# davrempe/contact-human-dynamics

Hardware: NVIDIA H100
Metric: optimised frames/sec (batched phys-optim) (higher is better)
Workload: dtype f64

## Files before the change

### contact-human-dynamics_b200/csrc/chd_api.cu

```cuda
#include <cuda_runtime.h>

#include <cstdio>
#include <cstdlib>
#include <cstring>
#include <vector>

#include "../../include/chd.h"
#include "chd_dev.h"

__global__ void chd_k_stage_begin(ChdDev D);
__global__ void chd_k_eval(ChdDev D);
__global__ void chd_k_init(ChdDev D);
__global__ void chd_k_kkt(ChdDev D);
__global__ void chd_k_kkt_gwin(ChdDev D);
__global__ void chd_k_kcopy(ChdDev D);
__global__ void chd_k_curv(ChdDev D);
__global__ void chd_k_asm(ChdDev D);
__global__ void chd_k_fp64_peak(int mode, int iters, double* sink);
__global__ void chd_k_hess_base(ChdDev D);
__global__ void chd_k_hess_dur(ChdDev D);
__global__ void chd_k_hess_zero(ChdDev D);
__global__ void chd_k_hess_fin(ChdDev D, int mode);
__global__ void chd_k_tables(ChdDev D);
__global__ void chd_k_clear_dyn(ChdDev D);
// ... 155 lines not shown
      chd_k_hess_dur<<<dim3(8, B), CHD_THREADS, 0, b->copy_stream>>>(b->D);
      chd_k_hess_fin<<<B, 128, 0, b->copy_stream>>>(b->D, 1);
      b->launches += 2;
    }
    chd_k_curv<<<dim3(8, B), 256, 0, b->copy_stream>>>(b->D);
    b->launches++;
    CHD_CUDA(cudaEventRecord(b->ev_copy, b->copy_stream));
    {
      Timer t(b, KT_SAMPLE);
      chd_k_snapshot<<<B, 128, 0, b->stream>>>(b->D, b->d_frames);
    }
    if ((it % check_every) == check_every - 1) {
      CHD_CUDA(cudaMemcpyAsync(b->h_ipm, b->D.ipm, B * sizeof(ChdIpm), cudaMemcpyDeviceToHost, b->stream));
      CHD_CUDA(cudaStreamSynchronize(b->stream));
      bool any = false;
      for (int i = 0; i < B; ++i) any |= (b->h_ipm[i].phase != CHD_PH_FINISHED);
      if (!any) break;
    }
  }
  CHD_CUDA(cudaMemcpyAsync(b->h_ipm, b->D.ipm, B * sizeof(ChdIpm), cudaMemcpyDeviceToHost, b->stream));
  CHD_CUDA(cudaStreamSynchronize(b->stream));
  CHD_CUDA(cudaStreamSynchronize(b->copy_stream));
  CHD_CUDA(cudaGetLastError());
  return 0;
}

}

extern "C" {

const char* chd_version(void) { return "libchd 0.1 (sm_90a)"; }

int chd_measure_fp64_peak(double* dfma_gflops, double* dmma_gflops) {
  int dev = 0, sms = 0;
  CHD_CUDA(cudaGetDevice(&dev));
  CHD_CUDA(cudaDeviceGetAttribute(&sms, cudaDevAttrMultiProcessorCount, dev));
  double* sink = nullptr;
  CHD_CUDA(cudaMalloc((void**)&sink, sizeof(double) * 1024));
  cudaEvent_t e0, e1;
  CHD_CUDA(cudaEventCreate(&e0));
  CHD_CUDA(cudaEventCreate(&e1));
  const int blocks = sms * 8, threads = 256, iters = 4096;
  for (int mode = 0; mode < 2; ++mode) {
    float best = 1e30f;
    for (int rep = 0; rep < 4; ++rep) {
      CHD_CUDA(cudaEventRecord(e0));
      chd_k_fp64_peak<<<blocks, threads>>>(mode, iters, sink);
      CHD_CUDA(cudaEventRecord(e1));
      CHD_CUDA(cudaEventSynchronize(e1));
      float ms = 0;
      CHD_CUDA(cudaEventElapsedTime(&ms, e0, e1));
      if (rep > 0 && ms < best) best = ms;
    }
    const double flop = mode == 0 ? (double)blocks * threads * iters * 8 * 2 : (double)blocks * (threads / 32) * iters * 4 * 512;
    double* out = mode == 0 ? dfma_gflops : dmma_gflops;
    if (out) *out = flop / (best * 1e-3) / 1e9;
  }
  cudaEventDestroy(e0), cudaEventDestroy(e1), cudaFree(sink);
  return 0;
}

static int batch_create_impl(const chd_phys_problem* problems, int32_t batch, const chd_phys_weights* weights, int32_t device,
                             const chd_phys_options& opt, chd_phys_batch* b);

int chd_phys_batch_create(const chd_phys_problem* problems, int32_t batch, const chd_phys_weights* weights, int32_t device,
                          const chd_phys_options* opt, chd_phys_batch** out) {
  if (!problems || batch <= 0 || !out) return -1;
  chd_phys_options o = {-1};
  if (opt) o = *opt;
  if (o.stage3_band_above < -1 || o.stage3_band_above > CHD_MAX_DUR) return -1;
  chd_phys_batch* b = new chd_phys_batch();
  std::memset(&b->D, 0, sizeof(b->D));
  const int rc = batch_create_impl(problems, batch, weights, device, o, b);
  if (rc) {
    chd_phys_batch_destroy(b);
    return rc;
  }
  *out = b;
  return 0;
}

static int batch_create_impl(const chd_phys_problem* problems, int32_t batch, const chd_phys_weights* weights, int32_t device,
                             const chd_phys_options& opt, chd_phys_batch* b) {
  const bool host_only = device == -2;
  if (device >= 0) CHD_CUDA(cudaSetDevice(device));
  chd_phys_weights w = {0.4, 1.7, 0.3, 0.1, 0.1};
  if (weights) w = *weights;
  int rc = chd_build_layout(problems, batch, w, b->hb, opt.stage3_band_above);
  if (rc) return rc;
  ChdHostBatch& hb = b->hb;
  ChdDev& D = b->D;
  std::memset(&D, 0, sizeof(D));
  b->host_only = host_only;
  if (host_only) return 0;
  D.B = hb.B, D.S = hb.S, D.Pmax = hb.Pmax, D.n_max = hb.n_max, D.m_max = hb.m_max, D.slots_max = hb.slots_max;
  D.sets_max = hb.sets_max, D.tab_max = hb.tab_max, D.F_max = hb.F_max, D.Kd_max = hb.Kd_max, D.Kr_max = hb.Kr_max;
  D.Na_max = hb.Na_max, D.nb_max = hb.nb_max, D.w_max = hb.w_max, D.par_stride = hb.par_stride(), D.n_ee_max = hb.n_ee_max;
  D.fo_max = hb.fo_max, D.Ph_max = hb.Ph_max;
  CHD_CUDA(cudaStreamCreate(&b->stream));
  {
    int dev_id = 0;
    cudaMemPool_t pool;
    CHD_CUDA(cudaGetDevice(&dev_id));
    CHD_CUDA(cudaDeviceGetDefaultMemPool(&pool, dev_id));
    unsigned long long keep = ~0ull;
    CHD_CUDA(cudaMemPoolSetAttribute(pool, cudaMemPoolAttrReleaseThreshold, &keep));
  }
// ... 174 lines not shown

int chd_phys_get_ent_col(const chd_phys_batch* b, int32_t* ent_col) {
  if (!b || !ent_col) return -1;
  if (b->host_only) {
    std::memcpy(ent_col, b->hb.ent_col.data(), b->hb.ent_col.size() * sizeof(int));
    return 0;
  }
  CHD_CUDA(cudaStreamSynchronize(b->stream));
  CHD_CUDA(cudaMemcpy(ent_col, b->D.ent_col, b->hb.ent_col.size() * sizeof(int), cudaMemcpyDeviceToHost));
  return 0;
}

int chd_phys_get_duals(const chd_phys_batch* b, double* y, double* zL, double* zU, double* s, double* row_scale, double* obj_scale) {
  if (!b || b->host_only) return -1;
  const size_t B = b->hb.B, mm = B * b->hb.m_max;
  CHD_CUDA(cudaStreamSynchronize(b->stream));
  if (y) CHD_CUDA(cudaMemcpy(y, b->D.y, mm * sizeof(double), cudaMemcpyDeviceToHost));
  if (zL) CHD_CUDA(cudaMemcpy(zL, b->D.zL, mm * sizeof(double), cudaMemcpyDeviceToHost));
  if (zU) CHD_CUDA(cudaMemcpy(zU, b->D.zU, mm * sizeof(double), cudaMemcpyDeviceToHost));
  if (s) CHD_CUDA(cudaMemcpy(s, b->D.s, mm * sizeof(double), cudaMemcpyDeviceToHost));
  if (row_scale) CHD_CUDA(cudaMemcpy(row_scale, b->D.sc, mm * sizeof(double), cudaMemcpyDeviceToHost));
  if (obj_scale) {
    std::vector<ChdIpm> ipm(B);
    CHD_CUDA(cudaMemcpy(ipm.data(), b->D.ipm, B * sizeof(ChdIpm), cudaMemcpyDeviceToHost));
    for (size_t i = 0; i < B; ++i) obj_scale[i] = ipm[i].sf;
  }
  return 0;
}

int chd_phys_stage_stats(const chd_phys_batch* b, double* stats) {
  if (!b || !stats || b->host_only || !b->h_ipm) return -1;
  const int B = b->hb.B;
  for (int s = 0; s < 6; ++s)
    for (int i = 0; i < B; ++i)
      for (int q = 0; q < 4; ++q) stats[((size_t)s * B + i) * 4 + q] = b->h_ipm[i].st_stat[s][q];
  return 0;
}

int chd_phys_solve_stage(chd_phys_batch* b, int32_t stage, int32_t max_iter, int32_t* status, int32_t* iters, double* stats) {
  if (!b || stage < 0 || stage > 5 || b->host_only) return -1;
  const int B = b->hb.B;
  int sched[1] = {stage};
  int rc = set_schedule(b, sched, 1, stage, max_iter);
  if (rc) return rc;
  if ((rc = run_schedule(b))) return rc;
  for (int i = 0; i < B; ++i) {
    const ChdIpm& I = b->h_ipm[i];
    if (status) status[i] = I.st_status[stage];
    if (iters) iters[i] = I.st_iters[stage];
    if (stats) {
      double* s = stats + 8 * i;
      s[0] = I.f, s[1] = I.E0, s[2] = I.viol_u, s[3] = I.dual_u, s[4] = I.compl_u, s[5] = I.mu, s[6] = I.delta_w, s[7] = I.ls_fail;
    }
    if (i == 0 && getenv("CHD_PROF")) fprintf(stderr, "chd prof (Mcycles) seq0 stage %d: err %.2f asm %.2f factor %.2f border %.2f back %.2f rec %.2f\n", stage, I.prof[0]/1e6, I.prof[1]/1e6, I.prof[2]/1e6, I.prof[3]/1e6, I.prof[4]/1e6, I.prof[5]/1e6);
  }
  return 0;
}

int chd_phys_sample_device(chd_phys_batch* b, double* out_device, void* stream) {
  if (!b || !out_device || b->host_only) return -1;
  cudaStream_t st = stream ? (cudaStream_t)stream : b->stream;
  if (st == b->stream) {
    Timer t(b, KT_SAMPLE);
    chd_k_sample<<<b->hb.B, 128, 0, st>>>(b->D, out_device, b->d_frames);
    return 0;
  }
  cudaEvent_t ev;
  CHD_CUDA(cudaEventCreateWithFlags(&ev, cudaEventDisableTiming));
  CHD_CUDA(cudaEventRecord(ev, b->stream));
  CHD_CUDA(cudaStreamWaitEvent(st, ev, 0));
  chd_k_sample<<<b->hb.B, 128, 0, st>>>(b->D, out_device, b->d_frames);
  CHD_CUDA(cudaEventRecord(ev, st));
  CHD_CUDA(cudaStreamWaitEvent(b->stream, ev, 0));
  CHD_CUDA(cudaEventDestroy(ev));
  return 0;
}

int chd_phys_sample(chd_phys_batch* b, double* out, int32_t* frames_out) {
  if (!b || !out || b->host_only) return -1;
  const ChdHostBatch& hb = b->hb;
  const size_t stride = 6 + 7 * (size_t)hb.n_ee_max, cnt = (size_t)hb.B * hb.fo_max * stride;
  CHD_CUDA(cudaMemsetAsync(b->d_samples, 0, cnt * sizeof(double), b->stream));
  int rc = chd_phys_sample_device(b, b->d_samples, nullptr);
  if (rc) return rc;
  CHD_CUDA(cudaMemcpyAsync(out, b->d_samples, cnt * sizeof(double), cudaMemcpyDeviceToHost, b->stream));
  if (frames_out) CHD_CUDA(cudaMemcpyAsync(frames_out, b->d_frames, hb.B * sizeof(int), cudaMemcpyDeviceToHost, b->stream));
  CHD_CUDA(cudaStreamSynchronize(b->stream));
  return 0;
}

int chd_phys_solve(chd_phys_batch* b, double* samples, int32_t* frames_out, int32_t* success, int32_t* stage_status,
                   int32_t* stage_iters) {
  if (!b || b->host_only) return -1;
  const ChdHostBatch& hb = b->hb;
  const int B = hb.B;
  const size_t stride = 6 + 7 * (size_t)hb.n_ee_max, snap = (size_t)B * hb.fo_max * stride;
  int sched[6] = {CHD_STAGE_11, CHD_STAGE_12, CHD_STAGE_21, CHD_STAGE_22, CHD_STAGE_3, CHD_STAGE_4};
  int rc = set_schedule(b, sched, 6, -1, 0);
  if (rc) return rc;
  if (samples) CHD_CUDA(cudaMemsetAsync(b->D.snapshots, 0, 3 * snap * sizeof(double), b->stream));
  if ((rc = run_schedule(b))) return rc;
  for (int i = 0; i < B; ++i) {
    const ChdIpm& I = b->h_ipm[i];
    if (success) success[2 * i] = I.st_status[CHD_STAGE_22] == 0, success[2 * i + 1] = I.st_status[CHD_STAGE_3] == 0 || I.st_status[CHD_STAGE_4] == 0;
    for (int s = 0; s < 6; ++s) {
      if (stage_status) stage_status[(size_t)s * B + i] = I.st_status[s];
      if (stage_iters) stage_iters[(size_t)s * B + i] = I.st_iters[s];
// ... 39 lines not shown
```

### contact-human-dynamics_b200/csrc/chd_kkt.cu

```cuda
#include <cuda_runtime.h>

#include "chd_block.cuh"
#include "chd_eval.cuh"
#include "chd_kkt_tiles.cuh"

__device__ __forceinline__ void chd_hess_sample(const ChdCtx& c, const ChdKT& K, const int* vk, int s, const ChdSpl* P, const double* sign, int np,
                                                int deriv, double wgt, int lane, double* ws) {
  const bool tau = c.opt_dur && s >= 2 && deriv == 0;
  if (lane < 28) {
    const int pa = lane / 14, q = lane % 14;
    double v0 = 0.0, v1 = 0.0, v2 = 0.0;
    int ia = -1;
    if (pa < np) {
      if (q < 12) {
        const int va = P[pa].var[q];
        const double wa = sign[pa] * chd_slot_w(P[pa], deriv, q);
        if (va >= 0 && wa != 0.0) {
          ia = vk[va];
          v0 = q % 3 == 0 ? wa : 0.0, v1 = q % 3 == 1 ? wa : 0.0, v2 = q % 3 == 2 ? wa : 0.0;
        }
      } else if (tau) {
        ChdTau u;
        chd_spl_tau(c, s, s - 2, P[pa], u);
        const int var = q == 12 ? u.va : u.vb;
// ... 434 lines not shown
  if (E0 <= CHD_TOL && violu <= CHD_CONSTR_VIOL_TOL && dual_u <= CHD_DUAL_INF_TOL && compl_u <= CHD_COMPL_INF_TOL) new_status = 0, done = true;
  else if (I.iter >= I.max_iter) new_status = -1, done = true;
  if (!done) {
    const double mu_min = fmin(CHD_TOL, CHD_COMPL_INF_TOL) / (CHD_KAPPA_EPS + 1.0);
    while (true) {
      const double Emu = fmax(fmax(dual_inf / s_d, cviol), compl_err(mu) / s_c);
      if (Emu <= CHD_KAPPA_EPS * mu && mu > mu_min) mu = fmax(mu_min, fmin(CHD_KAPPA_MU * mu, pow(mu, CHD_THETA_MU)));
      else break;
    }
  }
  __syncthreads();
  if (tid == 0) {
    I.f = D.cost[2 * b];
    I.E0 = E0, I.viol_u = violu, I.dual_u = dual_u, I.compl_u = compl_u;
    I.status = new_status;
    s_fail = 0;
    if (done) chd_stage_advance(D, I, new_status, c.sg.snap_after);
    if (!done) {
      I.mu = mu;
      I.tau = fmax(CHD_TAU_MIN, 1.0 - mu);
      if (I.iter == 0) I.theta_max = 1e4 * fmax(1.0, theta), I.theta_min = 1e-4 * fmax(1.0, theta), I.theta_ref = theta;
      if (mu != I.mu_filter) I.nfilt = 0, I.mu_filter = mu;
      I.theta0 = theta;
    }
  }
  if (done) return true;
  c.mu = mu;
  c.tau = fmax(CHD_TAU_MIN, 1.0 - mu);
  c.polish = E0 <= CHD_TOL && dual_u <= CHD_DUAL_INF_TOL && compl_u <= CHD_COMPL_INF_TOL && violu > CHD_CONSTR_VIOL_TOL &&
             I.delta_w < CHD_DW_POLISH;
  c.delta_w = c.polish ? CHD_DW_POLISH : I.delta_w;
  return false;
}

__device__ __forceinline__ void chd_kkt_assemble(const ChdDev& D, const ChdKktCtx& c) {
  const ChdIpm& I = *c.I;
  const ChdKT& K = c.K;
  const int tid = c.tid, nt = c.nt, n_act = c.n_act, nbl = c.nbl, nbt = c.nbt, nbp8 = c.nbp8, NBR = c.NBR, Na = K.Na;
  const int* vk = c.vk;
  const double mu = c.mu;
  if (c.polish) {
    const double extra = c.delta_w - I.delta_w;
    for (int i = tid; i < n_act; i += nt)
      if (vk[i] >= 0) chd_kadd(K, vk[i], vk[i], extra);
  }
  const double* r0 = D.rhs0 + (size_t)c.b * (D.Na_max + D.nb_max);
  const double* r1 = D.rhs1 + (size_t)c.b * (D.Na_max + D.nb_max);
  for (int i = tid; i < K.Np; i += nt)
    K.bord[((size_t)(i >> 3) * nbt + (NBR >> 3)) * 64 + (NBR & 7) * 8 + (i & 7)] = i < Na ? r0[i] + mu * r1[i] : 0.0;
  for (int i = tid; i < nbl; i += nt) K.corn[(size_t)NBR * nbp8 + i] = r0[D.Na_max + i] + mu * r1[D.Na_max + i];
}

template <class BandTile, class BordTile>
__device__ __forceinline__ void chd_kkt_update_compact(const ChdKktCtx& c, const unsigned short* s_pairs, unsigned char* cmp, const int* gnz,
                                                       int GB, int Gm, int tq, const BandTile& band_tile, const BordTile& bord_tile) {
  const int lane = c.lane, warp = c.warp, nbp8 = c.nbp8;
  const double *xpan = c.xpan, *ypan = c.ypan;
  int na;
  {
    const int g1 = lane + 32;
    const bool act0 = lane < Gm && (lane >= GB || lane < tq) && gnz[lane];
    const bool act1 = g1 < Gm && (g1 >= GB || g1 < tq) && gnz[g1 < 96 ? g1 : 0];
    const unsigned m0 = __ballot_sync(0xffffffffu, act0), m1 = __ballot_sync(0xffffffffu, act1);
    const unsigned below = (1u << lane) - 1u;
    const int n0 = __popc(m0);
    na = n0 + __popc(m1);
    if (act0) cmp[__popc(m0 & below)] = (unsigned char)lane;
    if (act1) cmp[n0 + __popc(m1 & below)] = (unsigned char)g1;
    __syncwarp();
  }
  auto corner = [&](const double* X, const double* Y, int bi, int bj) {
    double* Cc = c.cc + (size_t)(bi * 8 + (lane >> 2)) * nbp8 + bj * 8 + 2 * (lane & 3);
    double c0 = Cc[0], c1 = Cc[1];
    chd_tile_mma(c0, c1, X, Y, lane);
    Cc[0] = c0, Cc[1] = c1;
  };
  const int step = c.nwarp - 1, r8 = (lane >> 2) * 8 + 2 * (lane & 3);
  const int nb2 = (na + 1) >> 1, nblk = nb2 * (nb2 + 1) / 2;
  for (int p = warp - 1; p < nblk; p += step) {
    const int bi = s_pairs[p] >> 8, bj = s_pairs[p] & 255;
    const int i1 = 2 * bi + 1, j1 = 2 * bj + 1;
    const bool vi1 = i1 < na, vj1 = j1 < na;
    int gi[2], gj[2];
    gi[0] = cmp[2 * bi], gi[1] = cmp[i1 & 63];
    gj[0] = cmp[2 * bj], gj[1] = cmp[j1 & 63];
    double2 xf[2], yf[2];
    xf[0] = *reinterpret_cast<const double2*>(xpan + gi[0] * 64 + 2 * lane);
    yf[0] = *reinterpret_cast<const double2*>(ypan + gj[0] * 64 + 2 * lane);
    xf[1] = vi1 ? *reinterpret_cast<const double2*>(xpan + gi[1] * 64 + 2 * lane) : make_double2(0.0, 0.0);
    yf[1] = vj1 ? *reinterpret_cast<const double2*>(ypan + gj[1] * 64 + 2 * lane) : make_double2(0.0, 0.0);
    double* Cp[4];
    double2 cv[4];
#pragma unroll
    for (int t = 0; t < 4; ++t) {
      const int a = t & 1, cl = t >> 1;
      bool ok = (a == 0 || vi1) && (cl == 0 || vj1) && !(bi == bj && a == 0 && cl == 1);
      const int g_i = gi[a], g_j = gj[cl];
      ok = ok && !(g_i == 0 && g_j == 0);
      Cp[t] = nullptr;
      if (ok) {
        if (g_i < GB) Cp[t] = band_tile(g_i, g_j);
        else if (g_j < GB) Cp[t] = bord_tile(g_i - GB, g_j);
        else corner(xpan + g_i * 64, ypan + g_j * 64, g_i - GB, g_j - GB);
      }
      if (Cp[t]) cv[t] = *reinterpret_cast<const double2*>(Cp[t] + r8);
    }
#pragma unroll
    for (int t = 0; t < 4; ++t)
      if (Cp[t]) {
        const double2 xa = xf[t & 1], yb = yf[t >> 1];
        asm volatile("mma.sync.aligned.m8n8k4.row.col.f64.f64.f64.f64 {%0,%1}, {%2}, {%3}, {%0,%1};"
                     : "+d"(cv[t].x), "+d"(cv[t].y)
                     : "d"(-xa.x), "d"(yb.x));
      }
#pragma unroll
    for (int t = 0; t < 4; ++t)
      if (Cp[t]) {
        const double2 xa = xf[t & 1], yb = yf[t >> 1];
        asm volatile("mma.sync.aligned.m8n8k4.row.col.f64.f64.f64.f64 {%0,%1}, {%2}, {%3}, {%0,%1};"
                     : "+d"(cv[t].x), "+d"(cv[t].y)
                     : "d"(-xa.y), "d"(yb.y));
        *reinterpret_cast<double2*>(Cp[t] + r8) = cv[t];
      }
  }
}

template <class BandTile, class BordTile>
__device__ __forceinline__ void chd_kkt_update_wide(const ChdKktCtx& c, const unsigned short* s_pairs, const int* gnz, int GB, int npairs,
                                                    int tq, const BandTile& band_tile, const BordTile& bord_tile) {
  const int lane = c.lane, nwarp = c.nwarp, nbp8 = c.nbp8;
  const double *xpan = c.xpan, *ypan = c.ypan;
  double* cc = c.cc;
  const int r8 = (lane >> 2) * 8 + 2 * (lane & 3);
  int p = c.warp - 1;
  while (p < npairs) {
    struct { double* C; const double *X, *Y; } tl[4];
    int nq = 0;
    while (nq < 4 && p < npairs) {
      const int gi = s_pairs[p] >> 8, gj = s_pairs[p] & 255;
      p += nwarp - 1;
      if ((gi < GB && gi >= tq) || (gj < GB && gj >= tq) || !gnz[gi] || !gnz[gj]) continue;
      if (gi == 0 && gj == 0) continue;
      const double* X = xpan + gi * 64;
      const double* Y = ypan + gj * 64;
      if (gi < GB) {
        tl[nq].C = band_tile(gi, gj), tl[nq].X = X, tl[nq].Y = Y, ++nq;
      } else if (gj < GB) {
        tl[nq].C = bord_tile(gi - GB, gj), tl[nq].X = X, tl[nq].Y = Y, ++nq;
      } else {
        const int bi = gi - GB, bj = gj - GB;
        for (int e = lane; e < 64; e += 32) {
          const int r = e >> 3, cq = e & 7;
          double acc = 0.0;
#pragma unroll
          for (int kk = 0; kk < 8; ++kk) acc += X[r * 8 + kk] * Y[cq * 8 + kk];
          cc[(bi * 8 + r) * nbp8 + bj * 8 + cq] -= acc;
        }
      }
    }
    double c0[4], c1[4];
#pragma unroll
    for (int i = 0; i < 4; ++i)
      if (i < nq) c0[i] = tl[i].C[r8], c1[i] = tl[i].C[r8 + 1];
#pragma unroll
    for (int i = 0; i < 4; ++i)
      if (i < nq) {
        chd_tile_mma(c0[i], c1[i], tl[i].X, tl[i].Y, lane);
        tl[i].C[r8] = c0[i], tl[i].C[r8 + 1] = c1[i];
      }
  }
}

template <bool WS>
__device__ __forceinline__ void chd_kkt_factor(const ChdKktCtx& c, int& s_fail) {
  const ChdKT& K = c.K;
  const int tid = c.tid, nt = c.nt, lane = c.lane, warp = c.warp, nwarp = c.nwarp;
  const int Qs = c.Qs, Q = c.Q, nbt = c.nbt, nbp8 = c.nbp8, nbc = c.nbc, nbt_s = c.nbt_s;
  double *cc = c.cc, *ypan = c.ypan, *xpan = c.xpan, *dinv = c.dinv, *win = c.win, *bwin = c.bwin;
  for (int i = tid; i < nbp8 * nbp8; i += nt) cc[i] = K.corn[i];
  if (WS) {
    for (int idx = tid; idx < Q * Q * 64; idx += nt) {
      const int e = idx & 63, pr = idx >> 6, J = pr / Q, t = pr % Q;
      if (J + t < Q && J < nbc && J + t < nbc) win[chd_win_slot(J + t, J, Q) * 64 + e] = K.band[((size_t)J * Qs + t) * 64 + e];
    }
    for (int idx = tid; idx < Q * nbt * 64; idx += nt) {
      const int J = idx / (nbt * 64);
      if (J < nbc) bwin[idx] = K.bord[(size_t)J * nbt * 64 + idx % (nbt * 64)];
    }
  }
  __syncthreads();
  __shared__ int s_rs[2][96];
  __shared__ int s_gnz[2][96];
  constexpr int kPairs = WS ? 3000 : CHD_KKT_GROUPS_MAX * (CHD_KKT_GROUPS_MAX + 1) / 2;
  __shared__ unsigned short s_pairs[kPairs];
  __shared__ unsigned char s_cmp[CHD_KKT_THREADS / 32][64];
  __shared__ __align__(16) double s_winv[2][64];
  const int GB = K.q, Gm = K.q + nbt_s, npairs = Gm * (Gm + 1) / 2;
  for (int p = tid; p < npairs && p < kPairs; p += nt) {
    int gi = (int)((sqrt(8.0 * p + 1.0) - 1.0) * 0.5);
    while (gi * (gi + 1) / 2 > p) --gi;
    while ((gi + 1) * (gi + 2) / 2 <= p) ++gi;
    s_pairs[p] = (unsigned short)((gi << 8) | (p - gi * (gi + 1) / 2));
  }
  auto tri = [](int a_, int b_) { return a_ > b_ ? a_ * (a_ + 1) / 2 + b_ : b_ * (b_ + 1) / 2 + a_; };
  for (int g = tid; g < GB; g += nt) s_rs[0][g] = (1 + g) % Q;
  for (int g = tid; g < 96; g += nt) s_gnz[0][g] = 0, s_gnz[1][g] = 0;
  if (warp == 0) {
    const bool ok = chd_tile_ldl(WS ? win : K.band, dinv, s_winv[0], lane);
    if (!ok && lane == 0) s_fail = 1;
  }
  __syncthreads();
  int kslot = 0, cur = 0;
  for (int Kc = 0; Kc < nbc; ++Kc, cur ^= 1) {
    const int tq = min(K.q, nbc - 1 - Kc);
    const int* rs = s_rs[cur];
    auto band_tile = [&](int gi, int gj) -> double* {
      return WS ? win + (size_t)tri(rs[gi], rs[gj]) * 64 : K.band + ((size_t)(Kc + 1 + gj) * Qs + (gi - gj)) * 64;
    };
    auto bord_tile = [&](int bi, int gj) -> double* {
      return WS ? bwin + ((size_t)rs[gj] * nbt + bi) * 64 : K.bord + ((size_t)(Kc + 1 + gj) * nbt + bi) * 64;
    };
    double* Tkk = WS ? win + (size_t)tri(kslot, kslot) * 64 : K.band + (size_t)Kc * Qs * 64;
    double* Bk = WS ? bwin + (size_t)kslot * nbt * 64 : K.bord + (size_t)Kc * nbt * 64;
    const double* dv = dinv + 8 * cur;
    {
      const double* wv = s_winv[cur];
      const int r = lane >> 2, k = lane & 3;
      const double2 wf = *reinterpret_cast<const double2*>(wv + 2 * lane);
      const double d0 = dv[2 * k], d1 = dv[2 * k + 1];
      const int f0 = r * 8 + chd_frag_col(2 * k), f1 = r * 8 + chd_frag_col(2 * k + 1);
      for (int g = warp; g < tq + nbt_s; g += nwarp) {
        const bool band_t = g < tq;
        const int pg = band_t ? g : GB + (g - tq);
        const double* A = band_t ? (WS ? win + (size_t)tri(rs[g], kslot) * 64 : K.band + ((size_t)Kc * Qs + 1 + g) * 64) : Bk + (g - tq) * 64;
        const double ax = A[r * 8 + k], ay = A[r * 8 + k + 4];
        double c0 = 0.0, c1 = 0.0;
        asm volatile("mma.sync.aligned.m8n8k4.row.col.f64.f64.f64.f64 {%0,%1}, {%2}, {%3}, {%0,%1};"
                     : "+d"(c0), "+d"(c1)
                     : "d"(ax), "d"(wf.x));
        asm volatile("mma.sync.aligned.m8n8k4.row.col.f64.f64.f64.f64 {%0,%1}, {%2}, {%3}, {%0,%1};"
                     : "+d"(c0), "+d"(c1)
                     : "d"(ay), "d"(wf.y));
        const double x0 = c0 * d0, x1 = c1 * d1;
        ypan[pg * 64 + f0] = c0, ypan[pg * 64 + f1] = c1;
        xpan[pg * 64 + f0] = x0, xpan[pg * 64 + f1] = x1;
        double* G = band_t ? K.band + ((size_t)Kc * Qs + 1 + g) * 64 : K.bord + ((size_t)Kc * nbt + (g - tq)) * 64;
        *reinterpret_cast<double2*>(G + r * 8 + 2 * k) = make_double2(x0, x1);
        const bool nz = __any_sync(0xffffffffu, x0 != 0.0 || x1 != 0.0);
        if (lane == 0 && nz) s_gnz[cur][pg] = 1;
      }
    }
    if (WS)
      for (int e = tid; e < 64; e += nt) K.band[(size_t)Kc * Qs * 64 + e] = Tkk[e];
    __syncthreads();
    const int In = Kc + Q;
    if (WS && In < nbc) {
      for (int idx = tid - 32; idx < Q * 32 + nbt_s * 32; idx += nt - 32) {
        if (idx < 0) break;
        const int tile = idx >> 5, off = (idx & 31) * 2;
        if (tile < Q) {
          const int J = tile < GB ? Kc + 1 + tile : In;
          double* dst = tile < GB ? win + (size_t)tri(kslot, rs[tile]) * 64 : Tkk;
          chd_copy16(dst + off, K.band + ((size_t)J * Qs + (In - J)) * 64 + off, WS);
        } else {
          chd_copy16(Bk + (tile - Q) * 64 + off, K.bord + (size_t)In * nbt * 64 + (tile - Q) * 64 + off, WS);
        }
      }
    }
    if (warp == 0) {
      if (tq >= 1) {
        double* Tn = band_tile(0, 0);
        chd_tile_sub_xyT(Tn, xpan, ypan, lane);
        __syncwarp();
        const bool ok = chd_tile_ldl(Tn, dinv + 8 * (cur ^ 1), s_winv[cur ^ 1], lane);
        if (!ok && lane == 0) s_fail = 1;
      }
    } else {
      if (warp == 1) {
        for (int g = lane; g < GB; g += 32) {
          int v = kslot + 2 + g;
          while (v >= Q) v -= Q;
          s_rs[cur ^ 1][g] = v;
        }
        for (int g = lane; g < Gm; g += 32) s_gnz[cur ^ 1][g] = 0;
      }
      if (!WS && Gm > 64) chd_kkt_update_wide(c, s_pairs, s_gnz[cur], GB, npairs, tq, band_tile, bord_tile);
      else chd_kkt_update_compact(c, s_pairs, s_cmp[warp], s_gnz[cur], GB, Gm, tq, band_tile, bord_tile);
    }
    chd_copy_wait(WS);
    __syncthreads();
    kslot = kslot + 1 == Q ? 0 : kslot + 1;
  }
}

__device__ __forceinline__ void chd_kkt_border(const ChdDev& D, const ChdKktCtx& c, int& s_fail) {
  const int tid = c.tid, nt = c.nt, lane = c.lane, warp = c.warp, nbl = c.nbl, nbp8 = c.nbp8, NBR = c.NBR, Na = c.K.Na;
  double* cc = c.cc;
  for (int k = 0; k < nbl; ++k) {
    const double dk = cc[k * nbp8 + k];
    if (tid == 0 && !(dk > 0.0 && isfinite(dk))) s_fail = 1;
    __syncthreads();
    const double ik = 1.0 / dk;
    const int rem = nbl - k - 1;
    for (int idx = tid; idx < rem * rem; idx += nt) {
      const int i = k + 1 + idx / rem, j = k + 1 + idx % rem;
      if (j <= i) cc[i * nbp8 + j] -= cc[i * nbp8 + k] * ik * cc[j * nbp8 + k];
    }
    for (int j = k + 1 + tid; j < nbl; j += nt) cc[NBR * nbp8 + j] -= cc[j * nbp8 + k] * ik * cc[NBR * nbp8 + k];
    __syncthreads();
  }
  double* xb = c.xs + 8 * D.nbc_max;
  if (warp == 0) {
    for (int j = lane; j < nbl; j += 32) xb[j] = cc[NBR * nbp8 + j];
    __syncwarp();
    for (int k = nbl - 1; k >= 0; --k) {
      const double xk = xb[k] / cc[k * nbp8 + k];
      __syncwarp();
      for (int j = lane; j < k; j += 32) xb[j] -= cc[k * nbp8 + j] * xk;
      if (lane == 0) xb[k] = xk;
      __syncwarp();
    }
  }
  __syncthreads();
  for (int i = tid; i < nbl; i += nt) D.sol[(size_t)c.b * (D.Na_max + D.nb_max) + Na + i] = xb[i];
}

template <bool WS>
__device__ __forceinline__ void chd_kkt_backsub(const ChdDev& D, const ChdKktCtx& c) {
  const ChdKT& K = c.K;
  const int tid = c.tid, nt = c.nt, lane = c.lane, warp = c.warp, Q = c.Q, Qs = c.Qs, nbt = c.nbt, nbl = c.nbl, nbc = c.nbc;
  const int NBR = c.NBR, Na = K.Na;
  double *xs = c.xs, *sol = D.sol + (size_t)c.b * (D.Na_max + D.nb_max);
  const double* xb = xs + 8 * D.nbc_max;
  double* accv = c.xs2;
  for (int i = tid; i < K.Np; i += nt) {
    const double* bt = K.bord + (size_t)(i >> 3) * nbt * 64 + (i & 7);
    double v = bt[NBR * 8];
    for (int q2 = 0; q2 < nbl; ++q2) v -= bt[q2 * 8] * xb[q2];
    accv[i] = v;
  }
  const int per = Q * 64;
  const int R = max(1, (int)((c.win_region - (WS ? c.n_even + c.xs_len : 0)) / 64) / (2 * Q));
  double* stg = c.win;
  auto stage_chunk = [&](int Ktop, int buf, int t0, int tstep) {
    for (int idx = t0; idx < R * Q * 32; idx += tstep) {
// ... 169 lines not shown
  __syncthreads();
  chd_kkt_recover(D, c);
  CHD_PROF(5);
}
#undef CHD_PROF

__global__ void __launch_bounds__(256) chd_k_kcopy(ChdDev D) {
  const int b = blockIdx.y;
  if (!D.ipm[b].kw_req) return;
  if (blockIdx.x == 0) chd_rhs_clear(D, b);
  if (D.stages[D.ipm[b].stage].opt_dur && D.ipm[b].phase == CHD_PH_RUN) {
    chd_hess_clear(D, b, D.Kwork + (size_t)b * D.kstride, blockIdx.x, gridDim.x);
    return;
  }
  const size_t cnt2 = D.kstride / 2, per = (cnt2 + gridDim.x - 1) / gridDim.x;
  const size_t lo = (size_t)blockIdx.x * per, hi = lo + per < cnt2 ? lo + per : cnt2;
  const double2* src = reinterpret_cast<const double2*>(D.Kbase + (size_t)b * D.kstride);
  double2* dst = reinterpret_cast<double2*>(D.Kwork + (size_t)b * D.kstride);
  const size_t nt = blockDim.x;
  size_t i = lo + threadIdx.x;
  for (; i + 3 * nt < hi; i += 4 * nt) {
    const double2 v0 = src[i], v1 = src[i + nt], v2 = src[i + 2 * nt], v3 = src[i + 3 * nt];
    dst[i] = v0, dst[i + nt] = v1, dst[i + 2 * nt] = v2, dst[i + 3 * nt] = v3;
  }
  for (; i < hi; i += nt) dst[i] = src[i];
}

__global__ void __launch_bounds__(256) chd_k_curv(ChdDev D) {
  __shared__ double s_ws[8 * 192];
  const int b = blockIdx.y;
  const ChdIpm& I = D.ipm[b];
  if (!I.kw_req || I.phase != CHD_PH_RUN) return;
  ChdKT K;
  chd_kt_init(D, D.seq + b, D.Kwork + (size_t)b * D.kstride, K);
  K.ovf = &D.ipm[b].band_ovf;
  const int warp = threadIdx.x >> 5, lane = threadIdx.x & 31;
  chd_curv_rows(D, b, K, D.stages[I.stage], blockIdx.x * 8 + warp, gridDim.x * 8, lane, s_ws + warp * 192);
}

__global__ void __launch_bounds__(256) chd_k_asm(ChdDev D) {
  const int b = blockIdx.y;
  const ChdIpm& I = D.ipm[b];
  if (I.phase != CHD_PH_RUN) return;
  ChdKT K;
  chd_kt_init(D, D.seq + b, D.Kwork + (size_t)b * D.kstride, K);
  K.ovf = &D.ipm[b].band_ovf;
  if (!D.stages[I.stage].opt_dur) K.q = D.Qfix - 1;
  const size_t go = (size_t)b * (D.Na_max + D.nb_max);
  chd_assemble(D, b, K, I.delta_w, I.sf, blockIdx.x * blockDim.x + threadIdx.x, gridDim.x * blockDim.x, D.rhs0 + go, D.rhs1 + go);
}

__global__ void __launch_bounds__(256) chd_k_fp64_peak(int mode, int iters, double* sink) {
  const double s = 1.0 + 1e-9 * threadIdx.x;
  double a[8];
#pragma unroll
  for (int i = 0; i < 8; ++i) a[i] = 0.5 + i;
  if (mode == 0) {
    for (int it = 0; it < iters; ++it) {
#pragma unroll
      for (int i = 0; i < 8; ++i) a[i] = fma(a[i], s, 1e-3);
    }
  } else {
    const double x = s, y = 1.0 - 1e-9 * threadIdx.x;
    for (int it = 0; it < iters; ++it) {
#pragma unroll
      for (int i = 0; i < 4; ++i)
        asm volatile("mma.sync.aligned.m8n8k4.row.col.f64.f64.f64.f64 {%0,%1}, {%2}, {%3}, {%0,%1};"
                     : "+d"(a[2 * i]), "+d"(a[2 * i + 1])
                     : "d"(x), "d"(y));
    }
  }
  double t = 0;
#pragma unroll
  for (int i = 0; i < 8; ++i) t += a[i];
  if (t == 123.456) sink[threadIdx.x] = t;
}

__global__ void __launch_bounds__(CHD_KKT_THREADS) chd_k_kkt(ChdDev D) { chd_kkt_body<true>(D); }
__global__ void __launch_bounds__(CHD_KKT_THREADS) chd_k_kkt_gwin(ChdDev D) { chd_kkt_body<false>(D); }
```

### contact-human-dynamics_b200/csrc/chd_kkt_tiles.cuh

```cuda
#pragma once
#include "chd_dev.h"

struct ChdKT {
  int Na, Np, nbc, q, Q, nbt, nbp8;
  double *band, *bord, *corn;
  int* ovf;
};

__device__ __forceinline__ void chd_kt_init(const ChdDev& D, const ChdSeq* h, double* base, ChdKT& K) {
  K.Na = h->Na;
  K.Np = (h->Na + 7) & ~7;
  K.nbc = K.Np >> 3;
  K.Q = D.Q;
  K.q = D.Q - 1;
  K.nbt = D.nbt;
  K.nbp8 = 8 * D.nbt;
  K.ovf = nullptr;
  K.band = base;
  K.bord = base + (size_t)D.nbc_max * D.Q * 64;
  K.corn = K.bord + (size_t)D.nbc_max * D.nbt * 64;
}

__device__ __forceinline__ void chd_kadd(const ChdKT& K, int i, int j, double v) {
  if (i < j) { int t = i; i = j; j = t; }
  if (i < K.Na) {
    const int J = j >> 3;
    if ((i >> 3) - J > K.q) {
      if (K.ovf) *K.ovf = 1;
      return;
    }
    atomicAdd(K.band + ((size_t)J * K.Q + ((i >> 3) - J)) * 64 + (i & 7) * 8 + (j & 7), v);
  } else if (j < K.Na) {
    const int b = i - K.Na;
    atomicAdd(K.bord + ((size_t)(j >> 3) * K.nbt + (b >> 3)) * 64 + (b & 7) * 8 + (j & 7), v);
  } else {
    atomicAdd(K.corn + (size_t)(i - K.Na) * K.nbp8 + (j - K.Na), v);
  }
}
__device__ __forceinline__ double* chd_kdiag(const ChdKT& K, int k, bool band = false) {
  if (band || k < K.Na) return K.band + ((size_t)(k >> 3) * K.Q) * 64 + (k & 7) * 9;
  return K.corn + (size_t)(k - K.Na) * (K.nbp8 + 1);
}

__device__ __forceinline__ int chd_frag_col(int c) { return ((c & 3) << 1) | (c >> 2); }
__device__ __forceinline__ void chd_tile_mma(double& c0, double& c1, const double* X, const double* Y, int lane) {
  const double2 xa = *reinterpret_cast<const double2*>(X + 2 * lane);
  const double2 yb = *reinterpret_cast<const double2*>(Y + 2 * lane);
  asm volatile("mma.sync.aligned.m8n8k4.row.col.f64.f64.f64.f64 {%0,%1}, {%2}, {%3}, {%0,%1};"
               : "+d"(c0), "+d"(c1)
               : "d"(-xa.x), "d"(yb.x));
  asm volatile("mma.sync.aligned.m8n8k4.row.col.f64.f64.f64.f64 {%0,%1}, {%2}, {%3}, {%0,%1};"
               : "+d"(c0), "+d"(c1)
               : "d"(-xa.y), "d"(yb.y));
}
__device__ __forceinline__ void chd_tile_sub_xyT(double* C, const double* X, const double* Y, int lane) {
  const int r = lane >> 2, k = lane & 3;
  double c0 = C[r * 8 + 2 * k], c1 = C[r * 8 + 2 * k + 1];
  chd_tile_mma(c0, c1, X, Y, lane);
  C[r * 8 + 2 * k] = c0;
  C[r * 8 + 2 * k + 1] = c1;
}

__device__ __forceinline__ bool chd_tile_ldl(double* T, double* dinv, double* winv, int lane) {
  const int r = lane & 7;
  double a[8];
#pragma unroll
  for (int c = 0; c < 8; ++c) a[c] = c <= r ? T[r * 8 + c] : 0.0;
  bool ok = true;
  double w[8];
#pragma unroll
  for (int c = 0; c < 8; ++c) w[c] = c == r ? 1.0 : 0.0;
#pragma unroll
  for (int p = 0; p < 8; ++p) {
    const double dp = __shfl_sync(0xffffffffu, a[p], p, 8);
    ok = ok && (fabs(dp) > 1e-300) && isfinite(dp);
    const double inv = 1.0 / dp;
    const double lr = a[p] * inv;
#pragma unroll
    for (int c = p + 1; c < 8; ++c) {
      const double acp = __shfl_sync(0xffffffffu, a[p], c, 8);
      if (r >= c) a[c] -= lr * acp;
    }
    if (r > p) a[p] = lr;
    if (lane == p) dinv[p] = inv;
    if (p < 7) {
#pragma unroll
      for (int c = 0; c <= p; ++c) {
        const double wpc = __shfl_sync(0xffffffffu, w[c], p, 8);
        if (r > p) w[c] -= lr * wpc;
      }
    }
  }
  if (lane < 8) {
#pragma unroll
    for (int c = 0; c < 8; ++c)
      if (c <= r) T[r * 8 + c] = a[c];
  }
// ... 26 lines not shown
```

Before: 13180.

## Use m16n8k8 FP64 MMA for KKT trailing updates and panel solves

Replaces pairs of m8n8k4 double-precision MMAs with the larger m16n8k8 shape. Trailing-update tiles are grouped into 2x2 blocks handled by a shared helper, and the wide path now iterates over block pairs instead of queuing single tiles. The panel triangular solve processes two tiles per warp per MMA. The goal is fewer MMA instructions and better tensor-core throughput, at the cost of padded or zeroed work when blocks are half-empty and some extra corner-tile loads. It also adds optional clock-based profiling counters and updates the peak-FLOP probe to the new shape.

New measurement: 13780, median of 6. 4.5% higher.

```diff
diff --git a/contact-human-dynamics_b200/csrc/chd_api.cu b/contact-human-dynamics_b200/csrc/chd_api.cu
--- a/contact-human-dynamics_b200/csrc/chd_api.cu
+++ b/contact-human-dynamics_b200/csrc/chd_api.cu
@@ -231,7 +231,7 @@
       CHD_CUDA(cudaEventElapsedTime(&ms, e0, e1));
       if (rep > 0 && ms < best) best = ms;
     }
-    const double flop = mode == 0 ? (double)blocks * threads * iters * 8 * 2 : (double)blocks * (threads / 32) * iters * 4 * 512;
+    const double flop = mode == 0 ? (double)blocks * threads * iters * 8 * 2 : (double)blocks * (threads / 32) * iters * 4 * 2048;
     double* out = mode == 0 ? dfma_gflops : dmma_gflops;
     if (out) *out = flop / (best * 1e-3) / 1e9;
   }
@@ -512,7 +512,7 @@
       double* s = stats + 8 * i;
       s[0] = I.f, s[1] = I.E0, s[2] = I.viol_u, s[3] = I.dual_u, s[4] = I.compl_u, s[5] = I.mu, s[6] = I.delta_w, s[7] = I.ls_fail;
     }
-    if (i == 0 && getenv("CHD_PROF")) fprintf(stderr, "chd prof (Mcycles) seq0 stage %d: err %.2f asm %.2f factor %.2f border %.2f back %.2f rec %.2f\n", stage, I.prof[0]/1e6, I.prof[1]/1e6, I.prof[2]/1e6, I.prof[3]/1e6, I.prof[4]/1e6, I.prof[5]/1e6);
+    if (i == 0 && getenv("CHD_PROF")) fprintf(stderr, "chd prof (Mcycles) seq0 stage %d: err %.2f asm %.2f factor %.2f border %.2f back %.2f rec %.2f | factor (c): diag %.2f upd %.2f\n", stage, I.prof[0]/1e6, I.prof[1]/1e6, I.prof[2]/1e6, I.prof[3]/1e6, I.prof[4]/1e6, I.prof[5]/1e6, I.prof[6]/1e6, I.prof[7]/1e6);
   }
   return 0;
 }
diff --git a/contact-human-dynamics_b200/csrc/chd_kkt.cu b/contact-human-dynamics_b200/csrc/chd_kkt.cu
--- a/contact-human-dynamics_b200/csrc/chd_kkt.cu
+++ b/contact-human-dynamics_b200/csrc/chd_kkt.cu
@@ -510,10 +510,43 @@
 }
 
 template <class BandTile, class BordTile>
+__device__ __forceinline__ void chd_kkt_update_block(const ChdKktCtx& c, const int* gi, const int* gj, const bool* vi, const bool* vj, bool diag,
+                                                     int GB, const BandTile& band_tile, const BordTile& bord_tile) {
+  const int lane = c.lane;
+  const double2 z = make_double2(0.0, 0.0);
+  double2 xf[2], yf[2];
+#pragma unroll
+  for (int a = 0; a < 2; ++a) {
+    xf[a] = vi[a] ? *reinterpret_cast<const double2*>(c.xpan + gi[a] * 64 + 2 * lane) : z;
+    yf[a] = vj[a] ? *reinterpret_cast<const double2*>(c.ypan + gj[a] * 64 + 2 * lane) : z;
+  }
+  double* Cp[4];
+  double2 cv[4];
+#pragma unroll
+  for (int t = 0; t < 4; ++t) {
+    const int a = t & 1, cl = t >> 1;
+    bool ok = vi[a] && vj[cl] && !(diag && a == 0 && cl == 1);
+    ok = ok && !(gi[a] == 0 && gj[cl] == 0);
+    Cp[t] = nullptr;
+    if (ok) {
+      if (gi[a] < GB) Cp[t] = band_tile(gi[a], gj[cl]) + (lane >> 2) * 8 + 2 * (lane & 3);
+      else if (gj[cl] < GB) Cp[t] = bord_tile(gi[a] - GB, gj[cl]) + (lane >> 2) * 8 + 2 * (lane & 3);
+      else Cp[t] = c.cc + (size_t)((gi[a] - GB) * 8 + (lane >> 2)) * c.nbp8 + (gj[cl] - GB) * 8 + 2 * (lane & 3);
+    }
+    cv[t] = ok ? *reinterpret_cast<const double2*>(Cp[t]) : z;
+  }
+  const double2 xt = make_double2(-xf[0].x, -xf[0].y), xb = make_double2(-xf[1].x, -xf[1].y);
+#pragma unroll
+  for (int cl = 0; cl < 2; ++cl) chd_mma_16x8x8(cv[2 * cl], cv[2 * cl + 1], xt, xb, yf[cl]);
+#pragma unroll
+  for (int t = 0; t < 4; ++t)
+    if (Cp[t]) *reinterpret_cast<double2*>(Cp[t]) = cv[t];
+}
+
+template <class BandTile, class BordTile>
 __device__ __forceinline__ void chd_kkt_update_compact(const ChdKktCtx& c, const unsigned short* s_pairs, unsigned char* cmp, const int* gnz,
                                                        int GB, int Gm, int tq, const BandTile& band_tile, const BordTile& bord_tile) {
-  const int lane = c.lane, warp = c.warp, nbp8 = c.nbp8;
-  const double *xpan = c.xpan, *ypan = c.ypan;
+  const int lane = c.lane, warp = c.warp;
   int na;
   {
     const int g1 = lane + 32;
@@ -527,105 +560,28 @@
     if (act1) cmp[n0 + __popc(m1 & below)] = (unsigned char)g1;
     __syncwarp();
   }
-  auto corner = [&](const double* X, const double* Y, int bi, int bj) {
-    double* Cc = c.cc + (size_t)(bi * 8 + (lane >> 2)) * nbp8 + bj * 8 + 2 * (lane & 3);
-    double c0 = Cc[0], c1 = Cc[1];
-    chd_tile_mma(c0, c1, X, Y, lane);
-    Cc[0] = c0, Cc[1] = c1;
-  };
-  const int step = c.nwarp - 1, r8 = (lane >> 2) * 8 + 2 * (lane & 3);
+  const int step = c.nwarp - 1;
   const int nb2 = (na + 1) >> 1, nblk = nb2 * (nb2 + 1) / 2;
   for (int p = warp - 1; p < nblk; p += step) {
     const int bi = s_pairs[p] >> 8, bj = s_pairs[p] & 255;
     const int i1 = 2 * bi + 1, j1 = 2 * bj + 1;
-    const bool vi1 = i1 < na, vj1 = j1 < na;
-    int gi[2], gj[2];
-    gi[0] = cmp[2 * bi], gi[1] = cmp[i1 & 63];
-    gj[0] = cmp[2 * bj], gj[1] = cmp[j1 & 63];
-    double2 xf[2], yf[2];
-    xf[0] = *reinterpret_cast<const double2*>(xpan + gi[0] * 64 + 2 * lane);
-    yf[0] = *reinterpret_cast<const double2*>(ypan + gj[0] * 64 + 2 * lane);
-    xf[1] = vi1 ? *reinterpret_cast<const double2*>(xpan + gi[1] * 64 + 2 * lane) : make_double2(0.0, 0.0);
-    yf[1] = vj1 ? *reinterpret_cast<const double2*>(ypan + gj[1] * 64 + 2 * lane) : make_double2(0.0, 0.0);
-    double* Cp[4];
-    double2 cv[4];
-#pragma unroll
-    for (int t = 0; t < 4; ++t) {
-      const int a = t & 1, cl = t >> 1;
-      bool ok = (a == 0 || vi1) && (cl == 0 || vj1) && !(bi == bj && a == 0 && cl == 1);
-      const int g_i = gi[a], g_j = gj[cl];
-      ok = ok && !(g_i == 0 && g_j == 0);
-      Cp[t] = nullptr;
-      if (ok) {
-        if (g_i < GB) Cp[t] = band_tile(g_i, g_j);
-        else if (g_j < GB) Cp[t] = bord_tile(g_i - GB, g_j);
-        else corner(xpan + g_i * 64, ypan + g_j * 64, g_i - GB, g_j - GB);
-      }
-      if (Cp[t]) cv[t] = *reinterpret_cast<const double2*>(Cp[t] + r8);
-    }
-#pragma unroll
-    for (int t = 0; t < 4; ++t)
-      if (Cp[t]) {
-        const double2 xa = xf[t & 1], yb = yf[t >> 1];
-        asm volatile("mma.sync.aligned.m8n8k4.row.col.f64.f64.f64.f64 {%0,%1}, {%2}, {%3}, {%0,%1};"
-                     : "+d"(cv[t].x), "+d"(cv[t].y)
-                     : "d"(-xa.x), "d"(yb.x));
-      }
-#pragma unroll
-    for (int t = 0; t < 4; ++t)
-      if (Cp[t]) {
-        const double2 xa = xf[t & 1], yb = yf[t >> 1];
-        asm volatile("mma.sync.aligned.m8n8k4.row.col.f64.f64.f64.f64 {%0,%1}, {%2}, {%3}, {%0,%1};"
-                     : "+d"(cv[t].x), "+d"(cv[t].y)
-                     : "d"(-xa.y), "d"(yb.y));
-        *reinterpret_cast<double2*>(Cp[t] + r8) = cv[t];
-      }
+    const int gi[2] = {cmp[2 * bi], cmp[i1 & 63]}, gj[2] = {cmp[2 * bj], cmp[j1 & 63]};
+    const bool vi[2] = {true, i1 < na}, vj[2] = {true, j1 < na};
+    chd_kkt_update_block(c, gi, gj, vi, vj, bi == bj, GB, band_tile, bord_tile);
   }
 }
 
 template <class BandTile, class BordTile>
-__device__ __forceinline__ void chd_kkt_update_wide(const ChdKktCtx& c, const unsigned short* s_pairs, const int* gnz, int GB, int npairs,
+__device__ __forceinline__ void chd_kkt_update_wide(const ChdKktCtx& c, const unsigned short* s_pairs, const int* gnz, int GB, int Gm,
                                                     int tq, const BandTile& band_tile, const BordTile& bord_tile) {
-  const int lane = c.lane, nwarp = c.nwarp, nbp8 = c.nbp8;
-  const double *xpan = c.xpan, *ypan = c.ypan;
-  double* cc = c.cc;
-  const int r8 = (lane >> 2) * 8 + 2 * (lane & 3);
-  int p = c.warp - 1;
-  while (p < npairs) {
-    struct { double* C; const double *X, *Y; } tl[4];
-    int nq = 0;
-    while (nq < 4 && p < npairs) {
-      const int gi = s_pairs[p] >> 8, gj = s_pairs[p] & 255;
-      p += nwarp - 1;
-      if ((gi < GB && gi >= tq) || (gj < GB && gj >= tq) || !gnz[gi] || !gnz[gj]) continue;
-      if (gi == 0 && gj == 0) continue;
-      const double* X = xpan + gi * 64;
-      const double* Y = ypan + gj * 64;
-      if (gi < GB) {
-        tl[nq].C = band_tile(gi, gj), tl[nq].X = X, tl[nq].Y = Y, ++nq;
-      } else if (gj < GB) {
-        tl[nq].C = bord_tile(gi - GB, gj), tl[nq].X = X, tl[nq].Y = Y, ++nq;
-      } else {
-        const int bi = gi - GB, bj = gj - GB;
-        for (int e = lane; e < 64; e += 32) {
-          const int r = e >> 3, cq = e & 7;
-          double acc = 0.0;
-#pragma unroll
-          for (int kk = 0; kk < 8; ++kk) acc += X[r * 8 + kk] * Y[cq * 8 + kk];
-          cc[(bi * 8 + r) * nbp8 + bj * 8 + cq] -= acc;
-        }
-      }
-    }
-    double c0[4], c1[4];
-#pragma unroll
-    for (int i = 0; i < 4; ++i)
-      if (i < nq) c0[i] = tl[i].C[r8], c1[i] = tl[i].C[r8 + 1];
-#pragma unroll
-    for (int i = 0; i < 4; ++i)
-      if (i < nq) {
-        chd_tile_mma(c0[i], c1[i], tl[i].X, tl[i].Y, lane);
-        tl[i].C[r8] = c0[i], tl[i].C[r8 + 1] = c1[i];
-      }
+  auto live = [&](int g) { return g < Gm && (g >= GB || g < tq) && gnz[g]; };
+  const int nb2 = (Gm + 1) >> 1, nblk = nb2 * (nb2 + 1) / 2;
+  for (int p = c.warp - 1; p < nblk; p += c.nwarp - 1) {
+    const int bi = s_pairs[p] >> 8, bj = s_pairs[p] & 255;
+    const int gi[2] = {2 * bi, 2 * bi + 1}, gj[2] = {2 * bj, 2 * bj + 1};
+    const bool vi[2] = {live(gi[0]), live(gi[1])}, vj[2] = {live(gj[0]), live(gj[1])};
+    if (!(vi[0] || vi[1]) || !(vj[0] || vj[1])) continue;
+    chd_kkt_update_block(c, gi, gj, vi, vj, bi == bj, GB, band_tile, bord_tile);
   }
 }
 
@@ -653,7 +609,12 @@
   __shared__ unsigned short s_pairs[kPairs];
   __shared__ unsigned char s_cmp[CHD_KKT_THREADS / 32][64];
   __shared__ __align__(16) double s_winv[2][64];
-  const int GB = K.q, Gm = K.q + nbt_s, npairs = Gm * (Gm + 1) / 2;
+#ifdef CHD_PROFILE
+  __shared__ unsigned long long s_upd_end;
+  double prof_diag = 0.0, prof_upd = 0.0;
+  if (tid == 0) s_upd_end = 0;
+#endif
+  const int GB = K.q, Gm = K.q + nbt_s, nb2 = (Gm + 1) >> 1, npairs = nb2 * (nb2 + 1) / 2;
   for (int p = tid; p < npairs && p < kPairs; p += nt) {
     int gi = (int)((sqrt(8.0 * p + 1.0) - 1.0) * 0.5);
     while (gi * (gi + 1) / 2 > p) --gi;
@@ -683,35 +644,43 @@
     const double* dv = dinv + 8 * cur;
     {
       const double* wv = s_winv[cur];
-      const int r = lane >> 2, k = lane & 3;
+      const int r = lane >> 2, k = lane & 3, ng = tq + nbt_s;
       const double2 wf = *reinterpret_cast<const double2*>(wv + 2 * lane);
       const double d0 = dv[2 * k], d1 = dv[2 * k + 1];
       const int f0 = r * 8 + chd_frag_col(2 * k), f1 = r * 8 + chd_frag_col(2 * k + 1);
-      for (int g = warp; g < tq + nbt_s; g += nwarp) {
-        const bool band_t = g < tq;
-        const int pg = band_t ? g : GB + (g - tq);
-        const double* A = band_t ? (WS ? win + (size_t)tri(rs[g], kslot) * 64 : K.band + ((size_t)Kc * Qs + 1 + g) * 64) : Bk + (g - tq) * 64;
-        const double ax = A[r * 8 + k], ay = A[r * 8 + k + 4];
-        double c0 = 0.0, c1 = 0.0;
-        asm volatile("mma.sync.aligned.m8n8k4.row.col.f64.f64.f64.f64 {%0,%1}, {%2}, {%3}, {%0,%1};"
-                     : "+d"(c0), "+d"(c1)
-                     : "d"(ax), "d"(wf.x));
-        asm volatile("mma.sync.aligned.m8n8k4.row.col.f64.f64.f64.f64 {%0,%1}, {%2}, {%3}, {%0,%1};"
-                     : "+d"(c0), "+d"(c1)
-                     : "d"(ay), "d"(wf.y));
-        const double x0 = c0 * d0, x1 = c1 * d1;
-        ypan[pg * 64 + f0] = c0, ypan[pg * 64 + f1] = c1;
-        xpan[pg * 64 + f0] = x0, xpan[pg * 64 + f1] = x1;
-        double* G = band_t ? K.band + ((size_t)Kc * Qs + 1 + g) * 64 : K.bord + ((size_t)Kc * nbt + (g - tq)) * 64;
-        *reinterpret_cast<double2*>(G + r * 8 + 2 * k) = make_double2(x0, x1);
-        const bool nz = __any_sync(0xffffffffu, x0 != 0.0 || x1 != 0.0);
-        if (lane == 0 && nz) s_gnz[cur][pg] = 1;
+      for (int g0 = 2 * warp; g0 < ng; g0 += 2 * nwarp) {
+        double2 a[2], y[2];
+#pragma unroll
+        for (int h = 0; h < 2; ++h) {
+          const int g = g0 + h;
+          const double* A = g < tq ? (WS ? win + (size_t)tri(rs[g], kslot) * 64 : K.band + ((size_t)Kc * Qs + 1 + g) * 64) : Bk + (g - tq) * 64;
+          a[h] = g < ng ? make_double2(A[r * 8 + k], A[r * 8 + k + 4]) : make_double2(0.0, 0.0);
+          y[h] = make_double2(0.0, 0.0);
+        }
+        chd_mma_16x8x8(y[0], y[1], a[0], a[1], wf);
+#pragma unroll
+        for (int h = 0; h < 2; ++h) {
+          const int g = g0 + h;
+          if (g >= ng) break;
+          const bool band_t = g < tq;
+          const int pg = band_t ? g : GB + (g - tq);
+          const double x0 = y[h].x * d0, x1 = y[h].y * d1;
+          ypan[pg * 64 + f0] = y[h].x, ypan[pg * 64 + f1] = y[h].y;
+          xpan[pg * 64 + f0] = x0, xpan[pg * 64 + f1] = x1;
+          double* G = band_t ? K.band + ((size_t)Kc * Qs + 1 + g) * 64 : K.bord + ((size_t)Kc * nbt + (g - tq)) * 64;
+          *reinterpret_cast<double2*>(G + r * 8 + 2 * k) = make_double2(x0, x1);
+          const bool nz = __any_sync(0xffffffffu, x0 != 0.0 || x1 != 0.0);
+          if (lane == 0 && nz) s_gnz[cur][pg] = 1;
+        }
       }
     }
     if (WS)
       for (int e = tid; e < 64; e += nt) K.band[(size_t)Kc * Qs * 64 + e] = Tkk[e];
     __syncthreads();
     const int In = Kc + Q;
+#ifdef CHD_PROFILE
+    const long long tc0 = clock64();
+#endif
     if (WS && In < nbc) {
       for (int idx = tid - 32; idx < Q * 32 + nbt_s * 32; idx += nt - 32) {
         if (idx < 0) break;
@@ -733,6 +702,9 @@
         const bool ok = chd_tile_ldl(Tn, dinv + 8 * (cur ^ 1), s_winv[cur ^ 1], lane);
         if (!ok && lane == 0) s_fail = 1;
       }
+#ifdef CHD_PROFILE
+      if (lane == 0) prof_diag += (double)(clock64() - tc0);
+#endif
     } else {
       if (warp == 1) {
         for (int g = lane; g < GB; g += 32) {
@@ -742,13 +714,22 @@
         }
         for (int g = lane; g < Gm; g += 32) s_gnz[cur ^ 1][g] = 0;
       }
-      if (!WS && Gm > 64) chd_kkt_update_wide(c, s_pairs, s_gnz[cur], GB, npairs, tq, band_tile, bord_tile);
+      if (!WS && Gm > 64) chd_kkt_update_wide(c, s_pairs, s_gnz[cur], GB, Gm, tq, band_tile, bord_tile);
       else chd_kkt_update_compact(c, s_pairs, s_cmp[warp], s_gnz[cur], GB, Gm, tq, band_tile, bord_tile);
+#ifdef CHD_PROFILE
+      if (lane == 0) atomicMax(&s_upd_end, (unsigned long long)clock64());
+#endif
     }
     chd_copy_wait(WS);
     __syncthreads();
+#ifdef CHD_PROFILE
+    if (tid == 0) prof_upd += (double)((long long)s_upd_end - tc0);
+#endif
     kslot = kslot + 1 == Q ? 0 : kslot + 1;
   }
+#ifdef CHD_PROFILE
+  if (tid == 0) c.I->prof[6] += prof_diag, c.I->prof[7] += prof_upd;
+#endif
 }
 
 __device__ __forceinline__ void chd_kkt_border(const ChdDev& D, const ChdKktCtx& c, int& s_fail) {
@@ -1024,27 +1005,24 @@
 
 __global__ void __launch_bounds__(256) chd_k_fp64_peak(int mode, int iters, double* sink) {
   const double s = 1.0 + 1e-9 * threadIdx.x;
-  double a[8];
-#pragma unroll
-  for (int i = 0; i < 8; ++i) a[i] = 0.5 + i;
+  double2 a[8];
+#pragma unroll
+  for (int i = 0; i < 8; ++i) a[i] = make_double2(0.5 + i, 1.5 + i);
   if (mode == 0) {
     for (int it = 0; it < iters; ++it) {
 #pragma unroll
-      for (int i = 0; i < 8; ++i) a[i] = fma(a[i], s, 1e-3);
+      for (int i = 0; i < 8; ++i) a[i].x = fma(a[i].x, s, 1e-3);
     }
   } else {
-    const double x = s, y = 1.0 - 1e-9 * threadIdx.x;
+    const double2 x = make_double2(s, s), y = make_double2(1.0 - 1e-9 * threadIdx.x, 1.0);
     for (int it = 0; it < iters; ++it) {
 #pragma unroll
-      for (int i = 0; i < 4; ++i)
-        asm volatile("mma.sync.aligned.m8n8k4.row.col.f64.f64.f64.f64 {%0,%1}, {%2}, {%3}, {%0,%1};"
-                     : "+d"(a[2 * i]), "+d"(a[2 * i + 1])
-                     : "d"(x), "d"(y));
+      for (int i = 0; i < 4; ++i) chd_mma_16x8x8(a[2 * i], a[2 * i + 1], x, x, y);
     }
   }
   double t = 0;
 #pragma unroll
-  for (int i = 0; i < 8; ++i) t += a[i];
+  for (int i = 0; i < 8; ++i) t += a[i].x + a[i].y;
   if (t == 123.456) sink[threadIdx.x] = t;
 }
 
diff --git a/contact-human-dynamics_b200/csrc/chd_kkt_tiles.cuh b/contact-human-dynamics_b200/csrc/chd_kkt_tiles.cuh
--- a/contact-human-dynamics_b200/csrc/chd_kkt_tiles.cuh
+++ b/contact-human-dynamics_b200/csrc/chd_kkt_tiles.cuh
@@ -43,6 +43,13 @@
 }
 
 __device__ __forceinline__ int chd_frag_col(int c) { return ((c & 3) << 1) | (c >> 2); }
+
+__device__ __forceinline__ void chd_mma_16x8x8(double2& ct, double2& cb, double2 xt, double2 xb, double2 y) {
+  asm volatile("mma.sync.aligned.m16n8k8.row.col.f64.f64.f64.f64 {%0,%1,%2,%3}, {%4,%5,%6,%7}, {%8,%9}, {%0,%1,%2,%3};"
+               : "+d"(ct.x), "+d"(ct.y), "+d"(cb.x), "+d"(cb.y)
+               : "d"(xt.x), "d"(xb.x), "d"(xt.y), "d"(xb.y), "d"(y.x), "d"(y.y));
+}
+
 __device__ __forceinline__ void chd_tile_mma(double& c0, double& c1, const double* X, const double* Y, int lane) {
   const double2 xa = *reinterpret_cast<const double2*>(X + 2 * lane);
   const double2 yb = *reinterpret_cast<const double2*>(Y + 2 * lane);
```
